# mosure/bevy_gaussian_splatting

Measured on NVIDIA H100. Metric: rendered Msplats/sec @1080p, 6M-gaussian cloud, higher is better.
Workload: dtype f32 (f16-packed inputs)

## Files before the change

### bevy_gaussian_splatting_b200/csrc/radix.cu

```cuda
#include "common.cuh"
#include "launch.cuh"

namespace bgs {

constexpr int RS_THREADS = 512;
constexpr int RS_WARPS = RS_THREADS / 32;
constexpr int RS_TABLE_WORDS = RS_WARPS * 256;
constexpr int RS_MIN_CTAS = 2;
constexpr int LB_BATCH = 16;

constexpr unsigned long long ST_AGG = 1ull << 32, ST_INC = 2ull << 32;
__device__ __forceinline__ unsigned long long ld_status(const unsigned long long* p) {
    unsigned long long v;
    asm volatile("ld.relaxed.gpu.global.u64 %0, [%1];" : "=l"(v) : "l"(p) : "memory");
    return v;
}
__device__ __forceinline__ void st_status(unsigned long long* p, unsigned long long v) {
    asm volatile("st.relaxed.gpu.global.u64 [%0], %1;" ::"l"(p), "l"(v) : "memory");
}

struct SortParams {
    uint32_t* keys[2];
    uint32_t* vals[2];
    const uint32_t* n_ptr;
    uint32_t* hist;
    unsigned long long* status;
    size_t status_stride;
    uint32_t epoch;
    uint32_t* barrier;
    int passes;
    int shift0;
    int compute_hist;
    uint2* ranges;
};

constexpr size_t radix_smem_bytes(int items) {
    const size_t tile = (size_t)RS_THREADS * items;
    const size_t kv = tile > (size_t)RS_TABLE_WORDS ? tile : (size_t)RS_TABLE_WORDS;
    return (2 * kv + (size_t)RS_WARPS * 256 + 256 + 256 + 1024 + RS_WARPS) * 4;
}

template <int RS_ITEMS, bool MASK_TABLE>
__global__ void __launch_bounds__(RS_THREADS, RS_MIN_CTAS)
radix_coop_kernel(SortParams P) {
    constexpr int RS_TILE = RS_THREADS * RS_ITEMS;
    constexpr int KV_WORDS = RS_TILE > RS_TABLE_WORDS ? RS_TILE : RS_TABLE_WORDS;
    extern __shared__ __align__(16) uint32_t s_dyn[];
    uint32_t* s_keys = s_dyn;
    uint32_t* s_vals = s_keys + KV_WORDS;
    uint32_t (*s_whist)[256] = reinterpret_cast<uint32_t (*)[256]>(s_vals + KV_WORDS);
    uint32_t* s_binstart = &s_whist[0][0] + RS_WARPS * 256;
    uint32_t* s_gbase = s_binstart + 256;
    uint32_t* s_wtot = s_gbase + 256 + 1024;

    const int t = threadIdx.x, lane = t & 31, warp = t >> 5;
    const uint32_t G = gridDim.x;
    const uint32_t n = *P.n_ptr;
    const uint32_t num_tiles = (n + RS_TILE - 1) / RS_TILE;
    uint32_t bar_target = 0u;

    if (P.compute_hist) {
        uint32_t* s_hist = &s_whist[0][0];
        for (int i = t; i < P.passes * 256; i += RS_THREADS) s_hist[i] = 0u;
        __syncthreads();
        const uint32_t* kin = P.keys[0];
        for (uint32_t base = blockIdx.x * RS_TILE; base < n; base += G * RS_TILE) {
            uint32_t k[RS_ITEMS];
#pragma unroll
            for (int j = 0; j < RS_ITEMS; ++j) {
                const uint32_t i = base + j * RS_THREADS + t;
                k[j] = (i < n) ? __ldcg(kin + i) : 0u;
            }
            for (int p = 0; p < P.passes; ++p) {
                uint32_t run_d = 0xFFFFFFFFu, run_c = 0u;
#pragma unroll
                for (int j = 0; j < RS_ITEMS; ++j) {
                    const uint32_t i = base + j * RS_THREADS + t;
                    if (i >= n) break;
                    const uint32_t d = (k[j] >> (P.shift0 + 8 * p)) & 255u;
                    if (d == run_d) { ++run_c; }
                    else {
                        if (run_c) atomicAdd(&s_hist[p * 256 + run_d], run_c);
                        run_d = d; run_c = 1u;
                    }
                }
                if (run_c) atomicAdd(&s_hist[p * 256 + run_d], run_c);
            }
        }
        __syncthreads();
        for (int i = t; i < P.passes * 256; i += RS_THREADS) {
            const uint32_t c = s_hist[i];
            if (c) atomicAdd(&P.hist[i], c);
        }
        bar_target += G;
        grid_barrier(P.barrier, bar_target);
    }

    const unsigned long long ep = (unsigned long long)P.epoch << 34;
    int cur = 0;
    for (int p = 0; p < P.passes; ++p, cur ^= 1) {
        const int shift = P.shift0 + 8 * p;
        const uint32_t* __restrict__ keys_in = cur ? P.keys[1] : P.keys[0];
        const uint32_t* __restrict__ vals_in = cur ? P.vals[1] : P.vals[0];
        uint32_t* __restrict__ keys_out = cur ? P.keys[0] : P.keys[1];
        uint32_t* __restrict__ vals_out = cur ? P.vals[0] : P.vals[1];
        unsigned long long* status = P.status + (size_t)p * P.status_stride;
        const bool emit_ranges = P.ranges != nullptr && p == P.passes - 1;

        for (uint32_t tile = blockIdx.x; tile < num_tiles; tile += G) {
            const uint32_t tile_base = tile * RS_TILE;
            uint32_t k[RS_ITEMS];
            const uint32_t my_base = tile_base + warp * (32 * RS_ITEMS) + lane;
#pragma unroll
            for (int j = 0; j < RS_ITEMS; ++j) {
                const uint32_t i = my_base + j * 32;
                k[j] = (i < n) ? __ldcg(keys_in + i) : 0xFFFFFFFFu;
            }
#pragma unroll
            for (int i = 0; i < RS_WARPS * 256 / RS_THREADS; ++i) (&s_whist[0][0])[i * RS_THREADS + t] = 0u;
            if (MASK_TABLE) {
#pragma unroll
                for (int i = 0; i < RS_TABLE_WORDS / RS_THREADS; ++i) { s_vals[i * RS_THREADS + t] = 0u; s_keys[i * RS_THREADS + t] = 0u; }
            }
            __syncthreads();

            uint32_t rank[RS_ITEMS];
#pragma unroll
            for (int j = 0; j < RS_ITEMS; ++j) {
                const uint32_t d = (k[j] >> shift) & 255u;
                uint32_t peers, old;
                if (MASK_TABLE) {
                    uint32_t* mm = ((j & 1) ? s_keys : s_vals) + warp * 256;
                    atomicOr(&mm[d], 1u << lane);
                    __syncwarp();
                    peers = mm[d];
                    old = s_whist[warp][d];
                    __syncwarp();
                    if (lane == 31 - __clz(peers)) { mm[d] = 0u; s_whist[warp][d] = old + __popc(peers); }
                } else {
                    peers = __match_any_sync(0xffffffffu, d);
                    old = s_whist[warp][d];
                    __syncwarp();
                    if (lane == 31 - __clz(peers)) s_whist[warp][d] = old + __popc(peers);
                    __syncwarp();
                }
                rank[j] = old + __popc(peers & lanemask_lt());
            }
            __syncthreads();

            const uint32_t tile_end = tile_base + RS_TILE;
            const uint32_t pad = (tile_end > n) ? (tile_end - n) : 0u;
            uint32_t cnt = 0u, cnt_valid = 0u, incl = 0u, gh = 0u, gh_incl = 0u;
            unsigned long long* my_status = status + (size_t)tile * 256 + (t & 255);
            if (t < 256) {
#pragma unroll 8
                for (int w = 0; w < RS_WARPS; ++w) {
                    const uint32_t c = s_whist[w][t];
                    s_whist[w][t] = cnt;
                    cnt += c;
                }
                cnt_valid = (t == 255) ? cnt - pad : cnt;
                if (tile != 0) st_status(my_status, ep | ST_AGG | cnt_valid);
                incl = cnt;
#pragma unroll
                for (int o = 1; o < 32; o <<= 1) {
                    const uint32_t y = __shfl_up_sync(0xffffffffu, incl, o);
                    if (lane >= o) incl += y;
                }
                if (tile == 0) {
                    gh = __ldcg(P.hist + p * 256 + t);
                    gh_incl = gh;
#pragma unroll
                    for (int o = 1; o < 32; o <<= 1) {
                        const uint32_t y = __shfl_up_sync(0xffffffffu, gh_incl, o);
                        if (lane >= o) gh_incl += y;
                    }
                }
                if (lane == 31) { s_wtot[warp] = incl; s_wtot[8 + warp] = gh_incl; }
            }
            __syncthreads();
            uint32_t binstart = 0u, excl = 0u;
            if (t < 256) {
                uint32_t wprefix = 0u, gp = 0u;
                for (int w = 0; w < warp; ++w) { wprefix += s_wtot[w]; gp += s_wtot[8 + w]; }
                binstart = wprefix + incl - cnt;
                s_binstart[t] = binstart;
                if (tile == 0) {
                    excl = gp + gh_incl - gh;
                    st_status(my_status, ep | ST_INC | (excl + cnt_valid));
                }
            }
            __syncthreads();

#pragma unroll
            for (int j = 0; j < RS_ITEMS; ++j) {
                const uint32_t d = (k[j] >> shift) & 255u;
                const uint32_t i = my_base + j * 32;
                const uint32_t pos = rank[j] + s_binstart[d] + s_whist[warp][d];
                s_keys[pos] = k[j];
                s_vals[pos] = (i < n) ? __ldcg(vals_in + i) : 0u;
            }

            if (tile != 0) {
                uint32_t* s_part = s_binstart + 512;
                uint32_t* s_fnd = s_part + 512;
                const int d = t & 255, h = t >> 8;
                const unsigned long long* ps = status + (size_t)tile * 256 + d;
                bool done = false;
                for (uint32_t round = 0;; ++round) {
                    const uint32_t w0 = (2u * round + (uint32_t)h) * LB_BATCH;
                    uint32_t sum = 0u;
                    bool found = false;
                    if (!done) {
                        unsigned long long w[LB_BATCH];
#pragma unroll
                        for (int q = 0; q < LB_BATCH; ++q)
                            w[q] = (w0 + (uint32_t)q < tile) ? ld_status(ps - (size_t)256 * (w0 + q + 1)) : (ep | ST_INC);
#pragma unroll
                        for (int q = 0; q < LB_BATCH; ++q) {
                            if (!found) {
                                unsigned long long x = w[q];
                                while ((x >> 34) != (ep >> 34) || ((x >> 32) & 3ull) == 0ull) x = ld_status(ps - (size_t)256 * (w0 + q + 1));
                                sum += (uint32_t)x;
                                found = ((x >> 32) & 3ull) == 2ull;
                            }
                        }
                    }
                    s_part[h * 256 + d] = sum;
                    s_fnd[h * 256 + d] = found ? 1u : 0u;
                    __syncthreads();
                    if (!done) {
                        excl += s_part[d];
                        if (s_fnd[d]) done = true;
                        else { excl += s_part[256 + d]; done = s_fnd[256 + d] != 0u; }
                    }
                    if (__syncthreads_and(done ? 1 : 0)) break;
                }
                if (t < 256) st_status(my_status, ep | ST_INC | (excl + cnt_valid));
            }
            if (t < 256) s_gbase[t] = excl - binstart;
            __syncthreads();

            const uint32_t valid = RS_TILE - pad;
#pragma unroll 4
            for (uint32_t q = t; q < valid; q += RS_THREADS) {
                const uint32_t kk = s_keys[q];
                const uint32_t dst = s_gbase[(kk >> shift) & 255u] + q;
                keys_out[dst] = kk;
                vals_out[dst] = s_vals[q];
                if (emit_ranges) {
                    if (q == 0u || s_keys[q - 1] != kk) atomicMax(&P.ranges[kk].x, ~dst);
                    if (q == valid - 1u || s_keys[q + 1] != kk) atomicMax(&P.ranges[kk].y, dst + 1u);
                }
            }
            __syncthreads();
        }
        if (p + 1 < P.passes) {
            bar_target += G;
            grid_barrier(P.barrier, bar_target);
        }
    }
}

uint32_t radix_num_tiles(uint32_t capacity) {
    const uint32_t need = capacity / (RS_THREADS * 16u) + 1u;
    return need > 4096u ? need : 4096u;
}

namespace {
template <int ITEMS, bool MASK>
cudaError_t radix_launch_variant(const SortParams& P, uint32_t grid, cudaStream_t stream) {
    static bool attr_set[64] = {};
    const size_t smem = radix_smem_bytes(ITEMS);
    int dev = 0;
    cudaGetDevice(&dev);
    if (dev < 0 || dev >= 64 || !attr_set[dev]) {
        cudaError_t e = cudaFuncSetAttribute(radix_coop_kernel<ITEMS, MASK>, cudaFuncAttributeMaxDynamicSharedMemorySize, (int)smem);
        if (e != cudaSuccess) return e;
        if (dev >= 0 && dev < 64) attr_set[dev] = true;
    }
    SortParams p = P;
    void* args[] = {(void*)&p};
    return cudaLaunchCooperativeKernel((const void*)radix_coop_kernel<ITEMS, MASK>, dim3(grid), dim3(RS_THREADS), args, smem, stream);
}
}

int radix_coop_blocks_per_sm(int) {
    int b = 0;
    if (cudaFuncSetAttribute(radix_coop_kernel<16, false>, cudaFuncAttributeMaxDynamicSharedMemorySize, (int)radix_smem_bytes(16)) != cudaSuccess) return 0;
    if (cudaOccupancyMaxActiveBlocksPerMultiprocessor(&b, radix_coop_kernel<16, false>, RS_THREADS, radix_smem_bytes(16)) != cudaSuccess) return 0;
    return b;
}

cudaError_t launch_radix_sort(uint32_t* keys0, uint32_t* vals0, uint32_t* keys1, uint32_t* vals1, const uint32_t* n_ptr,
                              uint32_t capacity, uint32_t n_hint, uint32_t* hist, int compute_hist, void* status,
                              size_t status_stride, uint32_t epoch, uint32_t* barrier, int passes, int shift0, uint2* ranges,
                              int sm_count, int coop_per_sm, cudaStream_t stream) {
    SortParams P;
    P.keys[0] = keys0; P.keys[1] = keys1; P.vals[0] = vals0; P.vals[1] = vals1;
    P.n_ptr = n_ptr; P.hist = hist; P.status = reinterpret_cast<unsigned long long*>(status); P.status_stride = status_stride;
    P.epoch = epoch; P.barrier = barrier; P.passes = passes; P.shift0 = shift0; P.compute_hist = compute_hist;
    P.ranges = ranges;
    if (n_hint > capacity) n_hint = capacity;
    const uint64_t want = (uint64_t)n_hint + n_hint / 32 + 1024;
    uint32_t grid = (uint32_t)sm_count;
    auto items_for = [&](uint32_t g, uint32_t& waves) {
        const uint64_t per_wave = (uint64_t)g * RS_THREADS * 16u;
        waves = (uint32_t)((want + per_wave - 1) / per_wave);
        const uint64_t per_item = (uint64_t)g * RS_THREADS * waves;
        return (uint32_t)((want + per_item - 1) / per_item);
    };
    uint32_t waves = 1;
    uint32_t items = items_for(grid, waves);
    if (waves > 1 && coop_per_sm >= 2) {
        grid = 2u * (uint32_t)sm_count;
        items = items_for(grid, waves);
    }
    if (waves > 3) items = 17;
    const uint32_t rows = (uint32_t)(status_stride / 256);
    const uint32_t min_items = (uint32_t)(((uint64_t)capacity + (uint64_t)rows * RS_THREADS - 1) / ((uint64_t)rows * RS_THREADS));
    if (items < min_items) items = min_items;
    if (items <= 2) return radix_launch_variant<2, true>(P, grid, stream);
    if (items <= 4) return radix_launch_variant<4, true>(P, grid, stream);
    if (items <= 6) return radix_launch_variant<6, true>(P, grid, stream);
    if (items <= 8) return radix_launch_variant<8, true>(P, grid, stream);
    if (items <= 10) return radix_launch_variant<10, true>(P, grid, stream);
    if (items <= 12) return radix_launch_variant<12, true>(P, grid, stream);
    if (items <= 16) return radix_launch_variant<16, true>(P, grid, stream);
    return radix_launch_variant<16, false>(P, grid, stream);
}

}
```

Measured before the change: 17130.

## Seed decoupled lookback from both ends so final-wave tiles scan forward

```diff
diff --git a/bevy_gaussian_splatting_b200/csrc/radix.cu b/bevy_gaussian_splatting_b200/csrc/radix.cu
--- a/bevy_gaussian_splatting_b200/csrc/radix.cu
+++ b/bevy_gaussian_splatting_b200/csrc/radix.cu
@@ -9,7 +9,7 @@
 constexpr int RS_MIN_CTAS = 2;
 constexpr int LB_BATCH = 16;
 
-constexpr unsigned long long ST_AGG = 1ull << 32, ST_INC = 2ull << 32;
+constexpr unsigned long long ST_AGG = 1ull << 32, ST_INC = 2ull << 32, ST_EXC = 3ull << 32;
 __device__ __forceinline__ unsigned long long ld_status(const unsigned long long* p) {
     unsigned long long v;
     asm volatile("ld.relaxed.gpu.global.u64 %0, [%1];" : "=l"(v) : "l"(p) : "memory");
@@ -18,6 +18,17 @@
 __device__ __forceinline__ void st_status(unsigned long long* p, unsigned long long v) {
     asm volatile("st.relaxed.gpu.global.u64 [%0], %1;" ::"l"(p), "l"(v) : "memory");
 }
+
+#ifdef BGS_RADIX_STAMPS
+constexpr uint32_t RS_STAMP_TILES = 1024;
+__device__ unsigned long long g_rs_stamps[2][4][RS_STAMP_TILES][5];
+#define RS_STAMP(i)                                                                                              \
+    do {                                                                                                         \
+        if (t == 0 && tile < RS_STAMP_TILES && p < 4) g_rs_stamps[P.ranges != nullptr][p][tile][i] = clock64();  \
+    } while (0)
+#else
+#define RS_STAMP(i) do {} while (0)
+#endif
 
 struct SortParams {
     uint32_t* keys[2];
@@ -108,6 +119,7 @@
         const bool emit_ranges = P.ranges != nullptr && p == P.passes - 1;
 
         for (uint32_t tile = blockIdx.x; tile < num_tiles; tile += G) {
+            RS_STAMP(0);
             const uint32_t tile_base = tile * RS_TILE;
             uint32_t k[RS_ITEMS];
             const uint32_t my_base = tile_base + warp * (32 * RS_ITEMS) + lane;
@@ -150,6 +162,10 @@
 
             const uint32_t tile_end = tile_base + RS_TILE;
             const uint32_t pad = (tile_end > n) ? (tile_end - n) : 0u;
+            const uint32_t last = num_tiles - 1u;
+            const uint32_t last_wave = last - last % G;
+            const bool fwd = tile >= last_wave + (num_tiles - last_wave + 1u) / 2u;
+            const bool seed = tile == 0 || (fwd && tile == last);
             uint32_t cnt = 0u, cnt_valid = 0u, incl = 0u, gh = 0u, gh_incl = 0u;
             unsigned long long* my_status = status + (size_t)tile * 256 + (t & 255);
             if (t < 256) {
@@ -160,14 +176,14 @@
                     cnt += c;
                 }
                 cnt_valid = (t == 255) ? cnt - pad : cnt;
-                if (tile != 0) st_status(my_status, ep | ST_AGG | cnt_valid);
+                if (!seed) st_status(my_status, ep | ST_AGG | cnt_valid);
                 incl = cnt;
 #pragma unroll
                 for (int o = 1; o < 32; o <<= 1) {
                     const uint32_t y = __shfl_up_sync(0xffffffffu, incl, o);
                     if (lane >= o) incl += y;
                 }
-                if (tile == 0) {
+                if (seed) {
                     gh = __ldcg(P.hist + p * 256 + t);
                     gh_incl = gh;
 #pragma unroll
@@ -179,6 +195,7 @@
                 if (lane == 31) { s_wtot[warp] = incl; s_wtot[8 + warp] = gh_incl; }
             }
             __syncthreads();
+            RS_STAMP(1);
             uint32_t binstart = 0u, excl = 0u;
             if (t < 256) {
                 uint32_t wprefix = 0u, gp = 0u;
@@ -188,6 +205,9 @@
                 if (tile == 0) {
                     excl = gp + gh_incl - gh;
                     st_status(my_status, ep | ST_INC | (excl + cnt_valid));
+                } else if (seed) {
+                    excl = gp + gh_incl - cnt_valid;
+                    st_status(my_status, ep | ST_EXC | excl);
                 }
             }
             __syncthreads();
@@ -200,12 +220,16 @@
                 s_keys[pos] = k[j];
                 s_vals[pos] = (i < n) ? __ldcg(vals_in + i) : 0u;
             }
-
-            if (tile != 0) {
+            RS_STAMP(2);
+
+            if (!seed) {
                 uint32_t* s_part = s_binstart + 512;
                 uint32_t* s_fnd = s_part + 512;
                 const int d = t & 255, h = t >> 8;
                 const unsigned long long* ps = status + (size_t)tile * 256 + d;
+                const ptrdiff_t step = fwd ? 256 : -256;
+                const uint32_t reach = fwd ? last - tile : tile;
+                const unsigned long long want = fwd ? 3ull : 2ull;
                 bool done = false;
                 for (uint32_t round = 0;; ++round) {
                     const uint32_t w0 = (2u * round + (uint32_t)h) * LB_BATCH;
@@ -215,14 +239,14 @@
                         unsigned long long w[LB_BATCH];
 #pragma unroll
                         for (int q = 0; q < LB_BATCH; ++q)
-                            w[q] = (w0 + (uint32_t)q < tile) ? ld_status(ps - (size_t)256 * (w0 + q + 1)) : (ep | ST_INC);
+                            w[q] = (w0 + (uint32_t)q < reach) ? ld_status(ps + step * (ptrdiff_t)(w0 + q + 1)) : (ep | (want << 32));
 #pragma unroll
                         for (int q = 0; q < LB_BATCH; ++q) {
                             if (!found) {
                                 unsigned long long x = w[q];
-                                while ((x >> 34) != (ep >> 34) || ((x >> 32) & 3ull) == 0ull) x = ld_status(ps - (size_t)256 * (w0 + q + 1));
-                                sum += (uint32_t)x;
-                                found = ((x >> 32) & 3ull) == 2ull;
+                                while ((x >> 34) != (ep >> 34) || ((x >> 32) & 3ull) == 0ull) x = ld_status(ps + step * (ptrdiff_t)(w0 + q + 1));
+                                found = ((x >> 32) & 3ull) == want;
+                                sum += (fwd && !found) ? 0u - (uint32_t)x : (uint32_t)x;
                             }
                         }
                     }
@@ -236,10 +260,12 @@
                     }
                     if (__syncthreads_and(done ? 1 : 0)) break;
                 }
-                if (t < 256) st_status(my_status, ep | ST_INC | (excl + cnt_valid));
+                if (fwd) excl -= cnt_valid;
+                if (t < 256) st_status(my_status, fwd ? (ep | ST_EXC | excl) : (ep | ST_INC | (excl + cnt_valid)));
             }
             if (t < 256) s_gbase[t] = excl - binstart;
             __syncthreads();
+            RS_STAMP(3);
 
             const uint32_t valid = RS_TILE - pad;
 #pragma unroll 4
@@ -254,6 +280,7 @@
                 }
             }
             __syncthreads();
+            RS_STAMP(4);
         }
         if (p + 1 < P.passes) {
             bar_target += G;
@@ -261,6 +288,17 @@
         }
     }
 }
+
+#ifdef BGS_RADIX_STAMPS
+extern "C" int bgs_debug_radix_stamps(void* out, size_t bytes);
+extern "C" int bgs_debug_radix_stamps(void* out, size_t bytes) {
+    void* dev = nullptr;
+    if (bytes > sizeof(g_rs_stamps)) bytes = sizeof(g_rs_stamps);
+    if (cudaDeviceSynchronize() != cudaSuccess || cudaGetSymbolAddress(&dev, g_rs_stamps) != cudaSuccess) return 1;
+    if (out && cudaMemcpy(out, dev, bytes, cudaMemcpyDeviceToHost) != cudaSuccess) return 1;
+    return cudaMemset(dev, 0, sizeof(g_rs_stamps)) == cudaSuccess && cudaDeviceSynchronize() == cudaSuccess ? 0 : 1;
+}
+#endif
 
 uint32_t radix_num_tiles(uint32_t capacity) {
     const uint32_t need = capacity / (RS_THREADS * 16u) + 1u;
```

Result: no change. 17330, median of 6 (+1.1%).
